# SUSTech-SLAM-XYZZY/SurfelMapping

Measured on AMD Instinct MI355X. Metric: frames/sec per GPU, 1242x375 KITTI-shaped RGB-D+semantic, full associate+fuse+merge, higher is better.
Workload: dtype f32; 1 GPU; BASELINE configs[1]: KITTI 1242x375 synthetic street sequence, 0.8 m/frame, depth noise 15.0 mm, metricise+conflict+cull+splat+associate+fuse+append per frame; frames=5..6245, multi_gpu=single stream, surfels_start=157613, surfels_end=5487352

## Files before the change

### surfelmapping_amd/csrc/sm_api.hip

```cpp
#include "sm_ctx.h"
#include "sm_kernels.h"

#include <hip/hip_runtime.h>

#include <dirent.h>
#include <link.h>

#include <algorithm>
#include <chrono>
#include <cmath>
#include <cstdio>
#include <cstdlib>
#include <cstring>
#include <atomic>
#include <functional>
#include <memory>
#include <mutex>
#include <string>
#include <thread>
#include <vector>

using namespace sm;

namespace {
// ... 91 lines not shown
        bool here = false;
        while (struct dirent *qe = readdir(qd)) {
            if (qe->d_name[0] < '0' || qe->d_name[0] > '9') continue;
            char gp[400];
            snprintf(gp, sizeof gp, "%s/%s/gpuid", qdir, qe->d_name);
            FILE *fg = fopen(gp, "r");
            unsigned long g = 0;
            if (fg) { if (fscanf(fg, "%lu", &g) == 1 && g == gpuid) here = true; fclose(fg); }
            if (here) break;
        }
        closedir(qd);
        if (here) ++procs;
    }
    closedir(pd);
    return procs;
}

bool gpu_shared_with_other_process(int dev)
{
    static std::mutex mu;
    static std::chrono::steady_clock::time_point last[MAX_DEV];
    static int cached[MAX_DEV];
    static bool valid[MAX_DEV] = {};
    if (dev < 0 || dev >= MAX_DEV) return false;
    std::lock_guard<std::mutex> lk(mu);
    const auto now = std::chrono::steady_clock::now();
    if (!valid[dev] || std::chrono::duration_cast<std::chrono::milliseconds>(now - last[dev]).count() > 1000) {
        cached[dev] = kfd_processes_on_gpu(dev);
        last[dev] = now; valid[dev] = true;
    }
    return cached[dev] > 1;
}

bool compaction_needs_tickets(const sm_ctx *s)
{
    const int dev = s->cfg.device;
    if (s->sw.compact_tickets >= 0) return s->sw.compact_tickets != 0;
    if (dev < 0 || dev >= MAX_DEV) return true;
    {
        std::lock_guard<std::mutex> lk(g_compact_mu);
        if (g_ctx_on_dev[dev] > 1) return true;
    }
    return gpu_shared_with_other_process(dev);
}

Switches read_switches()
{
    Switches sw;
    auto off = [](const char *name) { const char *e = std::getenv(name); return e && e[0] == '0'; };
    auto num = [](const char *name, long unset) { const char *e = std::getenv(name); return e ? std::atol(e) : unset; };
    sw.defer_assoc = !off("SM_DEFER_ASSOC");
    sw.two_launch = !off("SM_TWO_LAUNCH");
    sw.tail_squeeze = !off("SM_TAIL_SQUEEZE");
    sw.tail_thresh = (uint32_t)std::max(1l, num("SM_TAIL_THRESH", (long)TAIL_DEAD_THRESH));
    sw.pass_split = (int)num("SM_PASS_SPLIT", 0);
    if (const char *e = std::getenv("SM_PASS_TRACE")) { sw.trace = true; sw.trace_prefix = e; }
    if (std::getenv("SM_COMPACT_TICKETS")) sw.compact_tickets = off("SM_COMPACT_TICKETS") ? 0 : 1;
    sw.capacity_wait_us = num("SM_CAPACITY_WAIT_US", 2000);
    sw.check_alive = std::getenv("SM_CHECK_ALIVE") != nullptr;
    if (std::getenv("SM_PASS_WG_PER_CU")) sw.pass_wg_per_cu = (int)std::max(1l, num("SM_PASS_WG_PER_CU", 1));
    if (std::getenv("SM_COMPACT_WG_PER_CU")) sw.compact_wg_per_cu = (int)std::max(1l, num("SM_COMPACT_WG_PER_CU", 1));
    return sw;
}

void resident_grids(const Switches &sw, int device, int *pass_grid, int *compact_grid)
{
    int cus = 0, per_cu = 0;
    if (hipDeviceGetAttribute(&cus, hipDeviceAttributeMultiprocessorCount, device) != hipSuccess || cus <= 0) return;
    if (hipOccupancyMaxActiveBlocksPerMultiprocessor(&per_cu, k_surfel_pass<1>, 256, 0) == hipSuccess && per_cu > 0) {
        const int want = sw.pass_wg_per_cu ? sw.pass_wg_per_cu : std::max(1, per_cu - 1);
        *pass_grid = std::max(256, std::min(cus * want, MAX_GRID));
    }
    if (hipOccupancyMaxActiveBlocksPerMultiprocessor(&per_cu, k_compact<true>, 256, 0) == hipSuccess && per_cu > 0) {
        const int want = sw.compact_wg_per_cu ? std::min(per_cu, sw.compact_wg_per_cu) : std::min(per_cu, 4);
        *compact_grid = std::max(1, cus * want);
    }
}

int alloc_set(SetBufs &b, size_t cap)
{
    return dalloc(b.pos_conf, cap) || dalloc(b.norm_rad, cap) || dalloc(b.color, cap) || dalloc(b.init_time, cap) ||
           dalloc(b.time, cap) ? SM_E_HIP : SM_OK;
}

int grid_surfels(const sm_ctx *s)
{
    return (int)std::min<uint64_t>(std::max<uint64_t>(s->slots.tiles(), 1), MAX_GRID);
}

void check_alive(sm_ctx *s, uint32_t stage)
{
    if (!s->d_chk) return;
    hipLaunchKernelGGL(k_check_alive, dim3(64), dim3(256), 0, s->stream, s->d_state, s->d_alive, s->d_tile_dead, s->d_chk, stage);
}

int take_error(sm_ctx *s)
{
    if (s->h_state->error != 0) {
        const int e = s->h_state->error;
        s->h_state->error = 0;
        HIPCK(hipMemcpyAsync(&s->d_state->error, &s->h_state->error, sizeof(int32_t), hipMemcpyHostToDevice, s->stream));
        HIPCK(hipStreamSynchronize(s->stream));
        g_err = e == SM_E_CAPACITY ? "model capacity (MAX_VERTICES) exceeded; frame's new surfels dropped"
              : e == SM_E_UNSUPPORTED ? "unsupported operation flagged on the device"
              : "device-side error";
        return e;
    }
    return SM_OK;
}


static inline uint32_t assoc_wgs(const sm_ctx *s)
{
    return (uint32_t)(s->n_pix_blocks + 1) / 2u;
}

int launch_fixup(sm_ctx *s, const FrameParams &fp, const FixArgs &x)
{
    hipLaunchKernelGGL(k_pass_fixup, dim3(x.n_crew + 1), dim3(256), 0, s->stream, s->M, s->d_state, fp, x);
    HIPCK(hipGetLastError());
    return SM_OK;
}

int launch_assoc(sm_ctx *s, const AssocArgs &a, uint32_t stage)
{
    hipLaunchKernelGGL((k_associate_direct<false>), dim3(assoc_wgs(s)), dim3(PIX_BLOCK), 0, s->stream, a, ShardArgs{});
// ... 222 lines not shown
    fpc.compact_tickets = compaction_needs_tickets(s) ? 1 : 0;
    const auto compact = splat ? k_compact<true> : k_compact<false>;
    hipLaunchKernelGGL(compact, dim3(grid), dim3(256), 0, s->stream, s->M, s->d_state, fpc, s->d_cm,
                       s->d_dm, s->d_zm, s->d_tile_cnt, s->d_tile_allow, s->d_tile_keep, s->keyT(), s->d_tile_flag, epoch,
                       s->d_group_base, s->d_tb, s->cur().tile_flags, s->part.d_compact, s->d_alive, s->d_tile_dead);
    HIPCK(hipGetLastError());
    if (s->tl.mark(s->stream, 4, timed)) return SM_E_HIP;
    return SM_OK;
}

int launch_post_fill(sm_ctx *s)
{
    hipLaunchKernelGGL(k_post_fill, dim3(1024), dim3(256), 0, s->stream, s->d_state, s->d_alive, s->d_tile_dead);
    HIPCK(hipGetLastError());
    check_alive(s, 4u + 16u * (uint32_t)(s->tick & 0xFFFF));
    return SM_OK;
}

int ss_compact(sm_ctx *s);

int launch_associate_only(sm_ctx *s, const FrameParams &fp)
{
    hipLaunchKernelGGL(k_associate, dim3(s->n_pix_blocks), dim3(PIX_BLOCK), 0, s->stream, s->M, s->d_state, fp,
                       s->cur().depthT, s->cur().rgbsT, s->keyT(), s->d_xs, s->d_ys, s->d_validmask, s->d_fusedmask, s->d_blk_cnt, s->d_tb);
    HIPCK(hipGetLastError());
    return SM_OK;
}

int launch_associate(sm_ctx *s, const FrameParams &fp, bool timed)
{
    int rc = launch_associate_only(s, fp);
    if (rc) return rc;
    if (s->tl.mark(s->stream, 5, timed) || s->tl.mark(s->stream, 6, timed)) return SM_E_HIP;
    const PassPartials::Fold f = s->part.fold();
    hipLaunchKernelGGL(k_append_scan, dim3(s->n_pix_blocks), dim3(PIX_BLOCK), 0, s->stream, s->M, s->d_state, fp, s->cur().depthT,
                       s->cur().rgbsT, s->d_xs, s->d_ys, s->d_validmask, s->d_fusedmask, s->d_blk_cnt, s->d_log, s->d_tb, f.compact,
                       f.n_compact, s->d_alive, s->d_tile_dead, s->d_stat, f.lazy, f.fix, f.n_fix);
    s->part.clear();
    s->slots.append_enqueued();
    HIPCK(hipGetLastError());
    if (s->tl.mark(s->stream, 7, timed)) return SM_E_HIP;
    check_alive(s, 5u + 16u * (uint32_t)(s->tick & 0xFFFF));
    return SM_OK;
}

int launch_squeeze(sm_ctx *s, bool in_frame, bool tail, bool timed)
{
    FrameParams fp = make_params(s, s->curr_pose);
    fp.maintenance = in_frame ? 2 : 1;
    fp.compact_now = 1;
    fp.conflict_cap = 0xFFFFFFFFu;
    fp.no_masks = 1;
    fp.tail_thresh = tail ? s->sw.tail_thresh : 0u;
    const uint64_t tiles = s->slots.tiles() + 1;
    const int ngroups = std::max<int>(1, (int)((tiles + GROUP - 1) / GROUP));
    hipLaunchKernelGGL(k_scan_cull, dim3(ngroups), dim3(1024), 0, s->stream, s->d_state, s->d_tile_cnt, s->d_tile_allow,
                       s->d_tile_keep, s->d_group_tot, s->d_tile_dead, 1u, fp.tail_thresh);
    hipLaunchKernelGGL(k_cull_finalize, dim3(1), dim3(1024), 0, s->stream, s->d_state, fp, s->d_cm, s->d_dm, s->d_zm,
                       s->d_tile_cnt, s->d_tile_allow, s->d_tile_keep, s->d_group_tot, s->d_group_base, s->d_conf_part, 0u,
                       s->d_alive, s->d_tile_dead, s->d_stat);
    if (!in_frame && s->slots.keys_are_slots())
        hipLaunchKernelGGL(k_remap_keys, dim3((s->P + 255) / 256), dim3(256), 0, s->stream, s->d_state, s->keyT(), s->P, s->d_alive,
                           s->d_tile_keep, s->d_group_base);
    HIPCK(hipGetLastError());
    if (s->tl.mark(s->stream, 2, timed) || s->tl.mark(s->stream, 3, timed)) return SM_E_HIP;
    return launch_compact(s, fp, false, timed);
}

int discard_model(sm_ctx *s)
{
    int rc = pull_state(s);
    if (rc) return rc;
    if (s->h_state->count == 0 && !s->slots.maybe_garbage() && s->h_state->conflict_count == 0 && s->h_state->visible_count == 0) return SM_OK;
    if (s->slots.maybe_garbage()) {
        HIPCK(hipMemsetAsync(s->d_alive, 0xFF, s->alive_words * 8, s->stream));
        HIPCK(hipMemsetAsync(s->d_tile_dead, 0, s->dead_tiles * 4, s->stream));
        s->slots.model_discarded();
    }
    s->h_state->conflict_count = 0; s->h_state->visible_count = 0;
    return publish_dense(s, 0, 0);
}

void end_frame(sm_ctx *s, bool timed = true)
{
    if (s->cfg.preprocess) std::swap(s->d_lastT, s->d_filteredT);
    memcpy(s->last_pose, s->curr_pose, 64);
    s->tl.end_frame(timed);
    s->tick++;
}

int begin_frame(sm_ctx *s, const uint8_t *d_rgb, const uint16_t *d_raw, const uint8_t *d_sem, const float *pose, bool tile_flags, bool carry,
                FrameParams *fp_out, uint32_t *n_prep)
{
    if (s->pending_cull) { g_err = "sm_stage_conflict without sm_stage_cull"; return SM_E_ARG; }
    memcpy(s->curr_pose, pose, 64);
    s->trk.note_pose(pose);
    FrameParams fp = make_params(s, pose);
    const bool fusing = s->ref_set && s->tick != 0;
    int rc;
    if ((rc = s->tl.mark(s->stream, 8, fusing))) return rc;
    if ((rc = s->tl.mark(s->stream, 0, fusing))) return rc;
    const bool will_splat = fusing;
    s->plane_set ^= 1;
    fp.par = s->plane_set;
    if (s->defer_ok && will_splat) s->key_set ^= 1;
    ChainArgs ca{};
// ... 2 lines not shown
        ca.border = (int)std::ceil(s->cfg.stereo_border - 0.5f);
        ca.do_movings = s->ref_set ? 1 : 0;
        if (s->ref_set) {
            float linv[16];
            invert4(s->last_pose, linv);
            mul4(linv, s->curr_pose, ca.t_c2l.m);
        }
    }
    if ((rc = launch_prep(s, d_rgb, d_raw, d_sem, fp, will_splat, tile_flags, carry, s->cfg.preprocess ? &ca : nullptr)) < 0) return rc;
    *n_prep = (uint32_t)rc;
    if (!s->ref_set) {
        if (s->cfg.preprocess) std::swap(s->d_lastT, s->d_filteredT);
        memcpy(s->last_pose, s->curr_pose, 64);
        s->ref_set = true;
        s->tick++;
        return 0;
    }
    if ((rc = s->tl.mark(s->stream, 1, fusing))) return rc;
    s->raw_valid = true;
    s->raw_tick = s->tick;
    if (s->tick == 0) {
        fp.init_mode = 1;
        fp.log_frame = 0;
        if ((rc = discard_model(s))) return rc;
        s->part.clear();
        s->part.n_compact = 0;
        if ((rc = launch_associate(s, fp, false))) return rc;
        end_frame(s, false);
        return 0;
    }
    fp.splat_follows = 1;
    fp.log_frame = 1;
    *fp_out = fp;
    return 1;
}

int enqueue_frame(sm_ctx *s, const uint8_t *d_rgb, const uint16_t *d_raw, const uint8_t *d_sem, const float *pose)
{
    if (s->ss_on) { g_err = "context is configured for sharding: use the sm_shard_* entry points"; return SM_E_ARG; }
    FrameParams fp;
    const bool fusing = s->ref_set && s->tick != 0 && !s->pending_cull;
    using Due = sm_slots::SlotSchedule::Due;
    const Due due = fusing ? s->slots.decide_due() : Due::forced;
    const bool compact_now = due != Due::none;
    const bool squeeze = fusing && due == Due::period && s->sw.tail_squeeze && s->defer_ok;
    const bool carry = fusing && s->defer_ok;
    int rc = SM_OK;
    uint32_t n_prep = 0;
    if (!carry && (rc = complete_held(s, false))) return rc;
    rc = begin_frame(s, d_rgb, d_raw, d_sem, pose, fusing && (!compact_now || squeeze), carry, &fp, &n_prep);
    if (rc <= 0) return rc;
    fp.compact_now = compact_now && !squeeze ? 1u : 0u;
    if (squeeze) {
        if ((rc = complete_held(s, true))) return rc;
        if ((rc = launch_squeeze(s, true, true, true))) return rc;
        s->slots.squeezed_in_frame();
    } else
        s->slots.cull_noted(fp.compact_now != 0u);
    s->slots.keys_drawn(fp.compact_now == 0u);
    const bool one_pass = !fp.compact_now;
    Timeline::Flags &fl = s->tl.frame();
    fl.compacted = !one_pass || squeeze; fl.one_pass = fl.direct = one_pass; fl.squeezed = squeeze;
    if (one_pass) {
        if ((rc = launch_surfel_pass(s, fp, true, true, n_prep, squeeze))) return rc;
        if ((rc = launch_associate_direct(s, fp, true))) return rc;
        end_frame(s);
        return SM_OK;
    }
    if ((rc = launch_conflict(s, fp, true))) return rc;
    if ((rc = launch_compact(s, fp, true, true))) return rc;
    if ((rc = launch_associate(s, fp, true))) return rc;
    end_frame(s);
    return SM_OK;
}

int upload_inputs(sm_ctx *s, const uint8_t *rgb, const uint16_t *depth, const uint8_t *sem)
{
    const size_t P = (size_t)s->P;
    hipStream_t st = s->stream;
    if (rgb) HIPCK(hipMemcpyAsync(s->d_rgb, rgb, P * 3, hipMemcpyHostToDevice, st));
    if (depth) HIPCK(hipMemcpyAsync(s->d_depth_raw, depth, P * 2, hipMemcpyHostToDevice, st));
    if (sem) HIPCK(hipMemcpyAsync(s->d_sem, sem, P, hipMemcpyHostToDevice, st));
    return SM_OK;
}

int alloc_frame_set(sm_ctx *s, FrameSet &f)
{
    auto get = [s](auto *&p, size_t n, bool zero) -> int {
        Dev<void> m;
        const size_t bytes = std::max<size_t>(n, 1) * sizeof *p;
        HIPCK(hipMalloc(m.put(), bytes));
        if (zero) HIPCK(hipMemset(m, 0, bytes));
        p = static_cast<std::remove_reference_t<decltype(p)>>(m.get());
        s->frame_mem.push_back(std::move(m));
        return SM_OK;
    };
    const size_t P = (size_t)s->P;
    return get(f.depthT, P, true) || get(f.rgbsT, P, true) || get(f.dcT, P, true) || get(f.tile_flags, s->tb_tiles, true) ||
           get(f.wave_cnt, s->dead_tiles, false) || get(f.prep_part, 256, false) ? SM_E_HIP : SM_OK;
}

int alloc_ctx(sm_ctx *s)
{
    const size_t P = (size_t)s->P, cap = s->cap, nwords = s->alive_words, ntiles = s->dead_tiles, tb = s->tb_tiles;
    if (hipStreamCreateWithFlags(s->stream.put(), hipStreamNonBlocking) != hipSuccess ||
        alloc_set(s->m_bufs[0], cap) ||
        dalloc(s->d_state, 1) || dalloc(s->d_log, FRAME_LOG_LEN) || hipHostMalloc(s->h_state.put(), sizeof(DevState), hipHostMallocDefault) != hipSuccess ||
        hipHostMalloc(s->h_stat.put(), 8, hipHostMallocMapped) != hipSuccess || hipHostGetDevicePointer((void **)&s->d_stat, s->h_stat, 0) != hipSuccess ||
        dalloc(s->d_filteredT, P) || dalloc(s->d_lastT, P) ||
        alloc_frame_set(s, s->fset[0]) || dalloc(s->d_key[0], P) ||
        (s->defer_ok && (alloc_frame_set(s, s->fset[1]) || dalloc(s->d_key[1], P))) ||
        dalloc(s->d_rgb, P * 3) || dalloc(s->d_sem, P) || dalloc(s->d_depth_raw, P) || dalloc(s->d_depth_f32, P) ||
        dalloc(s->d_xs, (size_t)s->W * 2) || dalloc(s->d_ys, (size_t)s->H * 2) ||
        dalloc(s->d_cm, nwords) || dalloc(s->d_dm, nwords) || dalloc(s->d_zm, nwords) ||
        dalloc(s->d_alive, nwords) || hipMemset(s->d_alive, 0xFF, nwords * 8) != hipSuccess ||
        dalloc(s->d_tile_dead, ntiles) || hipMemset(s->d_tile_dead, 0, ntiles * 4) != hipSuccess ||
        dalloc(s->d_tile_cnt, ntiles * 3) || dalloc(s->d_tile_allow, ntiles) || dalloc(s->d_tile_keep, ntiles) || dalloc(s->d_tile_flag, ntiles) ||
        hipMemset(s->d_tile_flag, 0, ntiles * 4) != hipSuccess ||
        dalloc(s->d_group_tot, (ntiles / GROUP + 2) * 4) || dalloc(s->d_group_base, ntiles / GROUP + 2) ||
        dalloc(s->d_conf_part, (size_t)MAX_GRID * 4) || dalloc(s->part.d_compact, (size_t)MAX_GRID) || dalloc(s->part.d_lazy, (size_t)MAX_GRID) ||
        dalloc(s->part.d_fix, (size_t)MAX_GRID * 2 + 2) || dalloc(s->d_undo, cap + TILE) ||
        dalloc(s->d_conf_sub, (size_t)2 * SUB_SET) || hipMemset(s->d_conf_sub, 0, (size_t)2 * SUB_SET * 4) != hipSuccess ||
        dalloc(s->d_tb, tb * 8) ||
        dalloc(s->d_validmask, (P + 63) / 64 + 4) || dalloc(s->d_fusedmask, (P + 63) / 64 + 4) || dalloc(s->d_blk_cnt, (size_t)s->n_pix_blocks) ||
        dalloc(s->d_blk_cand, (size_t)s->n_grp * CAND_GROUP_MAX) || dalloc(s->d_grp_cand, (size_t)s->n_grp) ||
        dalloc(s->d_frame_sub, (size_t)6 * SUB_SET) || hipMemset(s->d_frame_sub, 0, (size_t)6 * SUB_SET * 4) != hipSuccess)
        return SM_E_HIP;
    s->M.s[0] = s->m_bufs[0].view();
    *s->h_stat = 0ull;
    for (int i = 0; i < 2; ++i) { s->fset[i].nf_sub = s->d_frame_sub + (2 + 2 * i) * SUB_SET; s->fset[i].conf_sub = s->d_conf_sub + i * SUB_SET; }
    if (!s->defer_ok) s->alias_frame_sets();
    return SM_OK;
}

}


void sm_impl::invert4(const float *m, float *out)
{
    float a[16];
    a[0] = m[5] * m[10] * m[15] - m[5] * m[11] * m[14] - m[9] * m[6] * m[15] + m[9] * m[7] * m[14] +
           m[13] * m[6] * m[11] - m[13] * m[7] * m[10];
    a[4] = -m[4] * m[10] * m[15] + m[4] * m[11] * m[14] + m[8] * m[6] * m[15] - m[8] * m[7] * m[14] -
           m[12] * m[6] * m[11] + m[12] * m[7] * m[10];
    a[8] = m[4] * m[9] * m[15] - m[4] * m[11] * m[13] - m[8] * m[5] * m[15] + m[8] * m[7] * m[13] +
           m[12] * m[5] * m[11] - m[12] * m[7] * m[9];
    a[12] = -m[4] * m[9] * m[14] + m[4] * m[10] * m[13] + m[8] * m[5] * m[14] - m[8] * m[6] * m[13] -
            m[12] * m[5] * m[10] + m[12] * m[6] * m[9];
    a[1] = -m[1] * m[10] * m[15] + m[1] * m[11] * m[14] + m[9] * m[2] * m[15] - m[9] * m[3] * m[14] -
           m[13] * m[2] * m[11] + m[13] * m[3] * m[10];
    a[5] = m[0] * m[10] * m[15] - m[0] * m[11] * m[14] - m[8] * m[2] * m[15] + m[8] * m[3] * m[14] +
           m[12] * m[2] * m[11] - m[12] * m[3] * m[10];
    a[9] = -m[0] * m[9] * m[15] + m[0] * m[11] * m[13] + m[8] * m[1] * m[15] - m[8] * m[3] * m[13] -
           m[12] * m[1] * m[11] + m[12] * m[3] * m[9];
    a[13] = m[0] * m[9] * m[14] - m[0] * m[10] * m[13] - m[8] * m[1] * m[14] + m[8] * m[2] * m[13] +
            m[12] * m[1] * m[10] - m[12] * m[2] * m[9];
    a[2] = m[1] * m[6] * m[15] - m[1] * m[7] * m[14] - m[5] * m[2] * m[15] + m[5] * m[3] * m[14] +
           m[13] * m[2] * m[7] - m[13] * m[3] * m[6];
    a[6] = -m[0] * m[6] * m[15] + m[0] * m[7] * m[14] + m[4] * m[2] * m[15] - m[4] * m[3] * m[14] -
           m[12] * m[2] * m[7] + m[12] * m[3] * m[6];
    a[10] = m[0] * m[5] * m[15] - m[0] * m[7] * m[13] - m[4] * m[1] * m[15] + m[4] * m[3] * m[13] +
            m[12] * m[1] * m[7] - m[12] * m[3] * m[5];
    a[14] = -m[0] * m[5] * m[14] + m[0] * m[6] * m[13] + m[4] * m[1] * m[14] - m[4] * m[2] * m[13] -
            m[12] * m[1] * m[6] + m[12] * m[2] * m[5];
    a[3] = -m[1] * m[6] * m[11] + m[1] * m[7] * m[10] + m[5] * m[2] * m[11] - m[5] * m[3] * m[10] -
           m[9] * m[2] * m[7] + m[9] * m[3] * m[6];
    a[7] = m[0] * m[6] * m[11] - m[0] * m[7] * m[10] - m[4] * m[2] * m[11] + m[4] * m[3] * m[10] +
           m[8] * m[2] * m[7] - m[8] * m[3] * m[6];
    a[11] = -m[0] * m[5] * m[11] + m[0] * m[7] * m[9] + m[4] * m[1] * m[11] - m[4] * m[3] * m[9] -
// ... 929 lines not shown
```

### surfelmapping_amd/csrc/sm_ctx.h

```cpp
#pragma once

#include "../../include/sm_c_api.h"
#include "sm_device.h"
#include "sm_slots.h"

#include <hip/hip_runtime.h>

#include <algorithm>
#include <cassert>
#include <cmath>
#include <cstdio>
#include <cstring>
#include <functional>
#include <map>
#include <memory>
#include <string>
#include <utility>
#include <vector>

namespace sm { struct TrackState; struct TrackRgbState; struct RenderParams; struct ViewParams; struct ViewShade; struct RecallChunk; struct WarpChunk; }

namespace sm_impl __attribute__((visibility("hidden"))) {

using namespace sm;
// ... 154 lines not shown
    size_t cand_cap = 0;
    Event ev[2];
};

struct Lidar {
    Dev<float> d_dir, d_el;
    std::vector<float> key;
    Dev<uint8_t> d_poses;
    size_t pose_cap = 0;
    Dev<uint8_t> d_tally;
    Event ev[2];
    sm_lidar_stats_t stats{};
    bool stats_valid = false;
};

struct Place {
    bool on = false;
    sm_fern_params p{};
    Dev<uint4> d_table;
    Dev<uint8_t> d_rgb;
    Dev<uint16_t> d_depth;
    Dev<uint32_t> d_code;
    Dev<uint32_t> d_codes;
    Dev<int32_t> d_times;
    size_t cap = 0;
    std::vector<float> poses;
    std::vector<int32_t> times;
    Dev<unsigned long long> d_keys;
    Dev<uint32_t> d_dis;
    size_t dis_cap = 0;
    uint32_t count() const { return (uint32_t)times.size(); }
    bool timed = false;
    Event ev[4];
    bool auto_on = false;
    sm_auto_place_params ap{};
    int64_t rest_until = 0;
    sm_auto_place_stats_t stats{};
};

struct AutoLoop {
    bool on = false;
    bool search = false;
    sm_search_params sp{};
    sm_auto_loop_params p{};
    std::vector<std::string> paths;
    int64_t rest_until = 0;
    sm_auto_loop_stats_t stats{};
};

struct Switches {
    bool defer_assoc = true;
    bool two_launch = true;
    bool tail_squeeze = true;
    uint32_t tail_thresh = 0;
    int pass_split = 0;
    bool trace = false;
    std::string trace_prefix;
    int compact_tickets = -1;
    long capacity_wait_us = 2000;
    bool check_alive = false;
    int pass_wg_per_cu = 0;
    int compact_wg_per_cu = 0;
};

class HeldBack {
public:
    void hold_fixup(const FixArgs &x) { assert(!has_fix_ && !has_assoc_); fix_ = x; has_fix_ = true; }
    void hold_assoc(const AssocArgs &a) { assoc_ = a; has_assoc_ = true; }
    AssocArgs *take_assoc(FixArgs *&fix)
    {
        assert(has_assoc_ || !has_fix_);
        fix = std::exchange(has_fix_, false) ? &fix_ : nullptr;
        return std::exchange(has_assoc_, false) ? &assoc_ : nullptr;
    }
    void hold_settle(const ShardSettle &ss) { settle_ = ss; has_settle_ = true; }
    ShardSettle *take_settle() { return std::exchange(has_settle_, false) ? &settle_ : nullptr; }
    void hold_stats(uint32_t *nf) { nf_ = nf; }
    uint32_t *take_stats() { return std::exchange(nf_, nullptr); }
private:
    bool has_fix_ = false, has_assoc_ = false, has_settle_ = false;
    FixArgs fix_{};
    AssocArgs assoc_{};
    ShardSettle settle_{};
    uint32_t *nf_ = nullptr;
};

struct FrameSet {
    float *depthT = nullptr;
    uint32_t *rgbsT = nullptr;
    uint2 *dcT = nullptr;
    uint8_t *tile_flags = nullptr;
    uint4 *wave_cnt = nullptr;
    uint2 *prep_part = nullptr;
    uint32_t *nf_sub = nullptr;
    uint32_t *conf_sub = nullptr;
};

struct PassPartials {
    Dev<uint2> d_compact;
    Dev<uint4> d_lazy;
    Dev<uint2> d_fix;
    int fix_set = 0;
    uint32_t n_compact = 0;
    uint32_t n_fix = 0;
    bool pass_live = false;
    void clear() { pass_live = false; }
// ... 9 lines not shown
    uint64_t frames = 0, read = 0;
    int mark(hipStream_t st, int which, bool timed)
    {
        if (timed && ev) HIPCK(hipEventRecord(ev[which][frames % EV_RING], st));
        return SM_OK;
    }
    Flags &frame() { return flags[frames % EV_RING]; }
    void end_frame(bool timed) { if (timed && ev) frames++; }
};

}

using namespace sm_impl;

struct sm_ctx {
    Stream stream;
    Stream stream_in;
    sm_config cfg{};
    int W = 0, H = 0, P = 0;
    uint32_t cap = 0;
    int plane_set = 0;
    FrameSet fset[2];
    const FrameSet &cur() const { return fset[plane_set]; }
    const FrameSet &prev() const { return fset[plane_set ^ 1]; }
    void alias_frame_sets() { uint32_t *c = fset[1].conf_sub; fset[1] = fset[0]; fset[1].conf_sub = c; }
    Dev<uint64_t> d_key[2];
    int key_set = 0;
    uint64_t *keyT() const { return d_key[key_set]; }
    std::vector<Dev<void>> frame_mem;
    Model M{};
    SetBufs m_bufs[2];
    Dev<DevState> d_state;
    Host<DevState> h_state;
    Dev<float> d_filteredT, d_lastT;
    Dev<uint8_t> d_rgb, d_sem;
    Dev<uint16_t> d_depth_raw;
    static constexpr int IN_RING = 3;
    struct InSlot { Dev<uint8_t> rgb; uint8_t *sem = nullptr; uint16_t *depth = nullptr;
                    Host<unsigned char> h_stage; Event ev_in, ev_free; bool used = false; };
    InSlot in[IN_RING];
    size_t in_off_depth = 0, in_off_sem = 0, in_bytes = 0;
    uint32_t in_next = 0;
    const uint16_t *in_last_depth = nullptr; const uint8_t *in_last_sem = nullptr;
    int in_depth_slot = -1, in_sem_slot = -1;
    std::vector<std::pair<Host<unsigned char>, size_t>> pinned;
    Dev<float> d_depth_f32;
    Dev<float> d_xs, d_ys;
    float h_wtab[169];
    Dev<uint64_t> d_cm, d_dm, d_zm;
    Dev<uint32_t> d_tile_cnt, d_tile_allow, d_tile_keep, d_tile_flag;
    Dev<uint32_t> d_group_tot, d_group_base;
    Dev<uint64_t> d_alive;
    Dev<uint32_t> d_tile_dead;
    size_t alive_words = 0, dead_tiles = 0;
    sm_slots::SlotSchedule slots;
    Host<unsigned long long> h_stat; unsigned long long *d_stat = nullptr;
    Dev<uint32_t> d_tb;
    Dev<uint32_t> d_conf_part;
    PassPartials part;
    Dev<float> d_undo;
    int fix_grid = 128;
    Dev<uint32_t> d_blk_cand, d_grp_cand;
    Dev<uint32_t> d_frame_sub;
    uint32_t n_grp = 0, cand_group = 16;
    Dev<unsigned long long> d_pass_trace;
    int pass_trace_grid = 0;
    Dev<unsigned long long> d_ap_trace;
    int ap_trace_n[4] = {0, 0, 0, 0};
    Dev<uint32_t> d_conf_sub;
    uint32_t n_conf_part = 0;
    uint32_t tb_tiles = 0;
    int compact_grid = COMPACT_GRID;
    int pass_grid = MAX_GRID;
    Dev<uint64_t> d_validmask, d_fusedmask;
    Dev<uint2> d_blk_cnt;
    bool ss_on = false;
    bool rig_on = false;
    float rig_last_time = -1.0e30f;
    int ss_rank = 0, ss_world = 1;
    uint32_t ss_frames = 0;
    sm_collective_fn ss_coll = nullptr;
    void *ss_user = nullptr;
    void *ss_comm = nullptr;
    Dev<uint64_t> d_galive, d_new_alive, d_gmask;
    Dev<uint32_t> d_chk;
    Dev<uint64_t> d_capx;
    Dev<uint32_t> d_ss_info;
    Switches sw;
    bool defer_ok = false;
    HeldBack held;
    static constexpr uint32_t N_CREW = 32;
    int n_pix_blocks = 0;
    Dev<void> d_export;
    size_t export_bytes = 0;
    ModelView rm;
    Tracker trk;
    Retire ret;
    RenderMaps maps;
    Recall rec;
    Warp warp;
    AutoLoop aloop;
    Search srch;
    Lidar lid;
    Place place;
    int tick = 0;
    bool ref_set = false;
// ... 117 lines not shown
```

### surfelmapping_amd/csrc/sm_device.h

```cpp
#pragma once

#include <hip/hip_runtime.h>
#include <stdint.h>

namespace sm {

constexpr uint64_t KEY_EMPTY = 0x7FFFFFFFFFFFFFFFull;
constexpr int TILE = 1024;
constexpr int TILE_WORDS = TILE / 64;
constexpr int PIX_BLOCK = 256;
constexpr int SUB_STRIDE = 32;
constexpr int SUB_SET = 64 * SUB_STRIDE;

struct SurfelSet {
    float4 *pos_conf;
    float4 *norm_rad;
    uint32_t *color;
    float *init_time;
    float *time;
};

struct Model {
    SurfelSet s[2];
};

struct DevState {
    uint32_t count;
    uint32_t offset;
    uint32_t cur;
    uint32_t cull_n;
    uint32_t cull_src, cull_dst;
    uint32_t n_kill;
    uint32_t conflict_count;
    uint32_t data_count, unstable_count, fused_count;
    uint32_t visible_count;
    uint32_t append_n;
    int32_t error;
    uint32_t frames_logged;
    uint32_t n_static;
    uint32_t n_conf_skipped;
    uint32_t n_splat_skipped;
    uint32_t garbage;
    uint32_t garbage_prev;
    uint32_t do_compact;
    uint32_t cap_binds;
    uint32_t first_moving;
    uint32_t compact_ticket;
    uint32_t stat_frames;
    uint32_t first_live;
    uint32_t fl_dirty2[2];
    uint32_t slow_frames;
    uint32_t slow_done[2];
    uint32_t pend;
    uint32_t pend_tick;
    uint32_t holes_last;
    uint32_t sq_static;
    uint32_t sq_tail, sq_full;
};

struct FrameLog { uint32_t tick, n_before, n_after_cull, n_kill, conflict_count, visible_count, fused_count, unstable_count, n_static, n_conf_skipped, n_splat_skipped, n_slots; };
constexpr uint32_t FRAME_LOG_LEN = 1024;

struct FrameParams {
    float pose[16];
    float t_inv[16];
    float fx, fy, cx, cy;
    float inv_fx, inv_fy;
    float cols, rows;
    int W, H, P;
    float min_depth, max_depth;
    float conflict_thresh;
    float fuse_thresh;
    float stereo_border;
    int is_clean;
    int time;
    int time_delta;
    float depth_cutoff;
    uint32_t conflict_cap;
    int splat_follows;
    int log_frame;
    uint32_t max_vertices;
    int init_mode;
    float inv_fx_fb, inv_fy_fb;
    int use_bounds;
    uint32_t compact_now;
    int maintenance;
    int no_masks;
    uint32_t tail_thresh;
    int compact_tickets;
    int no_exempt;
    int shard_slots;
    int par;
};

__device__ __forceinline__ float min_glsl(float a, float b) { return (b < a) ? b : a; }

__device__ __forceinline__ int tex_idx(float t, int n)
{
    float f = floorf(t * (float)n);
    if (!(f >= 0.0f)) return 0;
    if (f > (float)(n - 1)) return n - 1;
    return (int)f;
}

__device__ __forceinline__ float3 xform3(const float *m, float x, float y, float z)
{
    float3 r;
    r.x = ((m[0] * x + m[4] * y) + m[8] * z) + m[12];
    r.y = ((m[1] * x + m[5] * y) + m[9] * z) + m[13];
    r.z = ((m[2] * x + m[6] * y) + m[10] * z) + m[14];
// ... 349 lines not shown
```

### surfelmapping_amd/csrc/sm_k_cull.h

```cpp
#pragma once

#ifndef SM_CONFLICT_WAVES
#define SM_CONFLICT_WAVES 5
#endif
__global__ __launch_bounds__(256) __attribute__((amdgpu_waves_per_eu(SM_CONFLICT_WAVES, 8))) void k_conflict(Model M, const DevState *__restrict__ st, FrameParams fp,
                                                  const uint2 *__restrict__ dcT ,
                                                  uint64_t *__restrict__ cm, uint64_t *__restrict__ dm,
                                                  uint64_t *__restrict__ zm, uint32_t *__restrict__ tile_cnt,
                                                  const uint32_t *__restrict__ tb, uint8_t *__restrict__ tile_flags,
                                                  uint32_t *__restrict__ blk_part ,
                                                  const uint64_t *__restrict__ alive,
                                                  uint32_t *__restrict__ conf_sub )
{
    __shared__ uint32_t s_red[4][3];
    __shared__ uint64_t s_m[3][TILE_WORDS];
    __shared__ uint8_t s_flags[64];
    const uint32_t N = st->count;
    const bool has_dead = st->garbage != 0u;
    const uint32_t exempt = fp.no_exempt ? 0xFFFFFFFFu : st->first_live;
    const float4 *__restrict__ pc = M.s[st->cur].pos_conf;
    const uint32_t ntiles = (N + TILE - 1) / TILE;
    const int lane = threadIdx.x & 63, wave = threadIdx.x >> 6;
    uint32_t skipped = 0;
    uint32_t acc = 0;
// ... 575 lines not shown
            if (threadIdx.x < 8) atomicExch(&tb[(size_t)tile * 8 + threadIdx.x], 0u);
            asm volatile("s_waitcnt vmcnt(0)" ::: "memory");
            __syncthreads();
            if (threadIdx.x == 0) {
                __hip_atomic_exchange(&tile_flag[tile], epoch, __ATOMIC_RELAXED, __HIP_MEMORY_SCOPE_AGENT);
                if (kcount && base_id != tile * TILE) {
                    const uint32_t first = base_id / TILE;
                    const uint32_t last = min(tile - 1u, (base_id + kcount - 1u) / TILE);
                    for (uint32_t t = first; t <= last; ++t) {
                        uint32_t spins = 0;
                        while (__hip_atomic_load(&tile_flag[t], __ATOMIC_RELAXED, __HIP_MEMORY_SCOPE_AGENT) != epoch) {
                            __builtin_amdgcn_s_sleep(2);
                            if (++spins > (1u << 24)) { st->error = -6; break; }
                        }
                    }
                }
            }
            __syncthreads();
            if (in_frame) {
                if (threadIdx.x < TILE_WORDS && (uint64_t)(tile * TILE_WORDS + threadIdx.x) * 64u < N) alive[tile * TILE_WORDS + threadIdx.x] = ~0ull;
                if (threadIdx.x == 0) { tile_dead[tile] = 0u; tile_flags[tile] = 0; }
            }
#pragma unroll
            for (int r = 0; r < 4; ++r) {
                if (kept[r]) {
                    set.pos_conf[nid[r]] = v[r];
                    set.norm_rad[nid[r]] = nr[r];
                    set.color[nid[r]] = col[r];
                    set.init_time[nid[r]] = it[r];
                    set.time[nid[r]] = tl[r];
                }
                bounds_expand_wave(tb, kept[r], nid[r] / (uint32_t)TILE, v[r].x, v[r].y, v[r].z, tl[r], false);
            }
        }
        if (SPLAT) {
#pragma unroll
            for (int r = 0; r < 4; ++r) {
                bool drew = false;
                if (kept[r])
                    drew = splat_one(fp, v[r].x, v[r].y, v[r].z, tl[r], nid[r], keyT);
                vis += (uint32_t)__popcll(__ballot(drew));
            }
        }
        __syncthreads();
    }
    if (SPLAT) {
        if (lane == 0) s_vis[wave] = vis;
        __syncthreads();
        if (threadIdx.x == 0)
            blk_part[blockIdx.x] = make_uint2(s_vis[0] + s_vis[1] + s_vis[2] + s_vis[3], skipped);
    }
}

__global__ __launch_bounds__(256) void k_cull_lazy(Model M, const DevState *__restrict__ st, FrameParams fp,
                                                   const uint64_t *__restrict__ cm, const uint64_t *__restrict__ dm,
                                                   const uint64_t *__restrict__ zm, const uint32_t *__restrict__ tile_cnt,
                                                   const uint32_t *__restrict__ tile_allow,
                                                   uint64_t *__restrict__ alive, uint32_t *__restrict__ tile_dead)
{
    const uint32_t N = st->cull_n;
    const SurfelSet set = M.s[st->cull_src];
    const uint32_t ntiles = (N + TILE - 1) / TILE;
    const int lane = threadIdx.x & 63, wave = threadIdx.x >> 6;
    const bool had_dead = st->garbage_prev != 0u, cap_binds = st->cap_binds != 0u;
    uint32_t iter = 0;
    uint32_t m_nconf = 0, m_nkill = 0, m_dead = 0;
    for (uint32_t tile = blockIdx.x; tile < ntiles; tile += gridDim.x, ++iter) {
        if ((iter & 63u) == 0u) {
            const uint64_t tl = (uint64_t)tile + (uint64_t)lane * gridDim.x;
            const bool in = tl < ntiles;
            const uint32_t tt = in ? (uint32_t)tl : 0u;
            m_nconf = tile_cnt[tt * 3]; m_nkill = tile_cnt[tt * 3 + 1];
            m_dead = had_dead ? tile_dead[tt] : 0u;
        }
        const int sl = (int)(iter & 63u);
        const uint32_t nconf = lane_bcast(m_nconf, sl), nkill = lane_bcast(m_nkill, sl);
        const uint32_t tdead = lane_bcast(m_dead, sl);
        const bool touched = nconf != 0u || nkill != 0u;
        if (!touched) continue;
        float4 pv[4];
#pragma unroll
        for (int r = 0; r < 4; ++r) {
            const uint32_t kc = min((tile * TILE_WORDS + r * 4 + wave) * 64u + lane, N - 1u);
            pv[r] = set.pos_conf[kc];
        }
        const uint32_t allow = (touched && cap_binds) ? tile_allow[tile] : nconf;
        uint32_t killed = 0;
#pragma unroll
        for (int r = 0; r < 4; ++r) {
            const int w = r * 4 + wave;
            const uint32_t word = tile * TILE_WORDS + (uint32_t)w;
            const uint32_t k = word * 64u + lane;
            const uint64_t base = (uint64_t)word * 64u;
            uint64_t range = 0ull;
            if (base < N) { const uint64_t rem = (uint64_t)N - base; range = rem >= 64 ? ~0ull : ((1ull << rem) - 1ull); }
            const uint64_t valid = range & ((tdead != 0u) ? alive[word] : ~0ull);
            uint64_t keep = valid, ce = 0ull;
            if (touched) {
                ce = cm[word];
                if (allow != nconf) {
                    uint32_t before = 0;
                    for (int x = 0; x < w; ++x) before += (uint32_t)__popcll(cm[tile * TILE_WORDS + x]);
                    ce = before >= allow ? 0ull : first_n_bits(ce, allow - before);
                }
                keep = ~(zm[word] | (ce & dm[word])) & valid;
                if (keep != valid && lane == 0) alive[word] = keep | ~range;
// ... 49 lines not shown
```

### surfelmapping_amd/csrc/sm_kernels.h

```cpp
#pragma once

#include "sm_device.h"

namespace sm {

#include "sm_k_prep.h"
#include "sm_k_cull.h"
#include "sm_k_pass.h"
#include "sm_k_assoc.h"
#include "sm_k_shard.h"

}
```

Before: 26350 frames/s.

## Fuse in-frame tail squeeze scan, cull finalize and compaction into one kernel

Adds a k_squeeze kernel that does the dead-tile prefix scan, the squeeze plan decision and the in-place compaction in one launch. Each block recomputes the per-tile dead prefix redundantly in LDS. Blocks order themselves with per-tile epoch flags and spin waits, and the last block finishes the frame bookkeeping. This replaces the scan_cull, cull_finalize and compact launch chain on in-frame squeeze frames, and lets the held frame completion skip its separate finalize. The aim is to cut launch count and global round trips, at the cost of redundant scanning per block, a large LDS footprint that may lower occupancy, and spin-wait deadlock risk. The compact grid is also capped by k_squeeze occupancy.

```diff
diff --git a/surfelmapping_amd/csrc/sm_api.hip b/surfelmapping_amd/csrc/sm_api.hip
--- a/surfelmapping_amd/csrc/sm_api.hip
+++ b/surfelmapping_amd/csrc/sm_api.hip
@@ -167,6 +167,7 @@
     sw.defer_assoc = !off("SM_DEFER_ASSOC");
     sw.two_launch = !off("SM_TWO_LAUNCH");
     sw.tail_squeeze = !off("SM_TAIL_SQUEEZE");
+    sw.squeeze_fused = !off("SM_SQUEEZE_FUSED");
     sw.tail_thresh = (uint32_t)std::max(1l, num("SM_TAIL_THRESH", (long)TAIL_DEAD_THRESH));
     sw.pass_split = (int)num("SM_PASS_SPLIT", 0);
     if (const char *e = std::getenv("SM_PASS_TRACE")) { sw.trace = true; sw.trace_prefix = e; }
@@ -187,6 +188,8 @@
         *pass_grid = std::max(256, std::min(cus * want, MAX_GRID));
     }
     if (hipOccupancyMaxActiveBlocksPerMultiprocessor(&per_cu, k_compact<true>, 256, 0) == hipSuccess && per_cu > 0) {
+        int per_cu_sq = 0;
+        if (hipOccupancyMaxActiveBlocksPerMultiprocessor(&per_cu_sq, k_squeeze, 256, 0) == hipSuccess && per_cu_sq > 0) per_cu = std::min(per_cu, per_cu_sq);
         const int want = sw.compact_wg_per_cu ? std::min(per_cu, sw.compact_wg_per_cu) : std::min(per_cu, 4);
         *compact_grid = std::max(1, cus * want);
     }
@@ -515,6 +518,18 @@
     fp.conflict_cap = 0xFFFFFFFFu;
     fp.no_masks = 1;
     fp.tail_thresh = tail ? s->sw.tail_thresh : 0u;
+    if (in_frame && s->sw.squeeze_fused) {
+        if (s->tl.mark(s->stream, 2, timed) || s->tl.mark(s->stream, 3, timed)) return SM_E_HIP;
+        s->part.clear();
+        const int grid = std::min(grid_surfels(s), s->compact_grid);
+        const uint32_t epoch = s->slots.next_cull_epoch();
+        fp.compact_tickets = compaction_needs_tickets(s) ? 1 : 0;
+        uint32_t *nf = s->held.take_stats();
+        hipLaunchKernelGGL(k_squeeze, dim3(grid), dim3(256), 0, s->stream, s->M, s->d_state, fp, s->d_tile_flag, epoch, s->d_tb,
+                           s->cur().tile_flags, s->d_alive, s->d_tile_dead, s->d_sq_sub, nf, s->part.fix_cur(), s->part.n_fix, s->d_log, s->d_stat);
+        HIPCK(hipGetLastError());
+        return s->tl.mark(s->stream, 4, timed) ? SM_E_HIP : SM_OK;
+    }
     const uint64_t tiles = s->slots.tiles() + 1;
     const int ngroups = std::max<int>(1, (int)((tiles + GROUP - 1) / GROUP));
     hipLaunchKernelGGL(k_scan_cull, dim3(ngroups), dim3(1024), 0, s->stream, s->d_state, s->d_tile_cnt, s->d_tile_allow,
@@ -623,7 +638,7 @@
     if (rc <= 0) return rc;
     fp.compact_now = compact_now && !squeeze ? 1u : 0u;
     if (squeeze) {
-        if ((rc = complete_held(s, true))) return rc;
+        if ((rc = complete_held(s, !s->sw.squeeze_fused))) return rc;
         if ((rc = launch_squeeze(s, true, true, true))) return rc;
         s->slots.squeezed_in_frame();
     } else
@@ -686,6 +701,7 @@
         dalloc(s->d_cm, nwords) || dalloc(s->d_dm, nwords) || dalloc(s->d_zm, nwords) ||
         dalloc(s->d_alive, nwords) || hipMemset(s->d_alive, 0xFF, nwords * 8) != hipSuccess ||
         dalloc(s->d_tile_dead, ntiles) || hipMemset(s->d_tile_dead, 0, ntiles * 4) != hipSuccess ||
+        dalloc(s->d_sq_sub, (size_t)SUB_SET) || hipMemset(s->d_sq_sub, 0, (size_t)SUB_SET * 4) != hipSuccess ||
         dalloc(s->d_tile_cnt, ntiles * 3) || dalloc(s->d_tile_allow, ntiles) || dalloc(s->d_tile_keep, ntiles) || dalloc(s->d_tile_flag, ntiles) ||
         hipMemset(s->d_tile_flag, 0, ntiles * 4) != hipSuccess ||
         dalloc(s->d_group_tot, (ntiles / GROUP + 2) * 4) || dalloc(s->d_group_base, ntiles / GROUP + 2) ||
diff --git a/surfelmapping_amd/csrc/sm_ctx.h b/surfelmapping_amd/csrc/sm_ctx.h
--- a/surfelmapping_amd/csrc/sm_ctx.h
+++ b/surfelmapping_amd/csrc/sm_ctx.h
@@ -230,6 +230,7 @@
     bool defer_assoc = true;
     bool two_launch = true;
     bool tail_squeeze = true;
+    bool squeeze_fused = true;
     uint32_t tail_thresh = 0;
     int pass_split = 0;
     bool trace = false;
@@ -345,6 +346,7 @@
     Dev<uint32_t> d_group_tot, d_group_base;
     Dev<uint64_t> d_alive;
     Dev<uint32_t> d_tile_dead;
+    Dev<uint32_t> d_sq_sub;
     size_t alive_words = 0, dead_tiles = 0;
     sm_slots::SlotSchedule slots;
     Host<unsigned long long> h_stat; unsigned long long *d_stat = nullptr;
diff --git a/surfelmapping_amd/csrc/sm_device.h b/surfelmapping_amd/csrc/sm_device.h
--- a/surfelmapping_amd/csrc/sm_device.h
+++ b/surfelmapping_amd/csrc/sm_device.h
@@ -56,6 +56,8 @@
     uint32_t holes_last;
     uint32_t sq_static;
     uint32_t sq_tail, sq_full;
+    uint32_t sq_done;
+    uint32_t sq_ticket;
 };
 
 struct FrameLog { uint32_t tick, n_before, n_after_cull, n_kill, conflict_count, visible_count, fused_count, unstable_count, n_static, n_conf_skipped, n_splat_skipped, n_slots; };
diff --git a/surfelmapping_amd/csrc/sm_k_cull.h b/surfelmapping_amd/csrc/sm_k_cull.h
--- a/surfelmapping_amd/csrc/sm_k_cull.h
+++ b/surfelmapping_amd/csrc/sm_k_cull.h
@@ -651,6 +651,223 @@
     }
 }
 
+constexpr uint32_t SQ_SLAB = 8192;
+static_assert(TAIL_GARBAGE_DIV == sm_squeeze::GARBAGE_DIV, "one garbage rule");
+
+__device__ __forceinline__ void finalize_frame(DevState *__restrict__ st, uint32_t *__restrict__ nf, const uint2 *__restrict__ fix_prev,
+                                               uint32_t n_fix_prev, FrameLog *__restrict__ log, uint32_t *s_red);
+
+__global__ __launch_bounds__(256) void k_squeeze(Model M, DevState *__restrict__ st, FrameParams fp,
+                                                 uint32_t *__restrict__ tile_flag, uint32_t epoch,
+                                                 uint32_t *__restrict__ tb, uint8_t *__restrict__ tile_flags,
+                                                 uint64_t *__restrict__ alive, uint32_t *__restrict__ tile_dead,
+                                                 uint32_t *__restrict__ done_sub ,
+                                                 uint32_t *__restrict__ nf, const uint2 *__restrict__ fix_prev, uint32_t n_fix_prev,
+                                                 FrameLog *__restrict__ log, unsigned long long *__restrict__ host_stat)
+{
+    __shared__ uint32_t s_slab[SQ_SLAB];
+    __shared__ uint32_t s_pre[sm_squeeze::THREADS];
+    __shared__ uint32_t s_wsum[4], s_first, s_dense, s_left, s_tk, s_last, s_red[16];
+    __shared__ uint64_t s_keep[TILE_WORDS];
+    __shared__ uint32_t s_kpre[TILE_WORDS + 1];
+    const uint32_t N = st->count;
+    const SurfelSet set = M.s[st->cur];
+    const uint32_t ntiles = (N + TILE - 1) / TILE;
+    const int lane = threadIdx.x & 63, wave = threadIdx.x >> 6;
+    const uint32_t C = sm_squeeze::chunk_len(ntiles);
+    const uint32_t t0 = min(threadIdx.x * C, ntiles), t1 = min(t0 + C, ntiles);
+    sm_squeeze::Chunk ch = sm_squeeze::chunk_empty();
+    if (threadIdx.x == 0) { s_first = sm_squeeze::NONE; s_dense = sm_squeeze::NONE; s_left = 0u; }
+    for (uint32_t s0 = 0; s0 < ntiles; s0 += SQ_SLAB) {
+        const uint32_t s1 = min(s0 + SQ_SLAB, ntiles);
+        {
+            uint32_t d[SQ_SLAB / 256];
+#pragma unroll
+            for (int u = 0; u < (int)(SQ_SLAB / 256); ++u) d[u] = tile_dead[min(s0 + (uint32_t)u * 256u + threadIdx.x, ntiles - 1u)];
+#pragma unroll
+            for (int u = 0; u < (int)(SQ_SLAB / 256); ++u) {
+                const uint32_t i = s0 + (uint32_t)u * 256u + threadIdx.x;
+                if (i < s1) s_slab[i - s0] = d[u];
+            }
+        }
+        __syncthreads();
+        for (uint32_t t = max(t0, s0); t < min(t1, s1); ++t) {
+            const uint32_t d = s_slab[t - s0];
+            s_slab[t - s0] = ch.dead;
+            sm_squeeze::chunk_add(ch, t, d, fp.tail_thresh);
+        }
+        __syncthreads();
+    }
+    const uint32_t slab0 = ntiles ? ((ntiles - 1u) / SQ_SLAB) * SQ_SLAB : 0u;
+    uint32_t inc = ch.dead;
+#pragma unroll
+    for (int o = 1; o < 64; o <<= 1) {
+        const uint32_t x = __shfl_up(inc, o);
+        if (lane >= o) inc += x;
+    }
+    if (lane == 63) s_wsum[wave] = inc;
+    __syncthreads();
+    uint32_t pre = inc - ch.dead;
+    for (int w = 0; w < wave; ++w) pre += s_wsum[w];
+    s_pre[threadIdx.x] = pre;
+    if (ch.first_dead != sm_squeeze::NONE) atomicMin(&s_first, ch.first_dead);
+    if (ch.first_dense != sm_squeeze::NONE) atomicMin(&s_dense, ch.first_dense);
+    __syncthreads();
+    sm_squeeze::Totals tot;
+    tot.dead = s_wsum[0] + s_wsum[1] + s_wsum[2] + s_wsum[3];
+    tot.first_dead = s_first; tot.first_dense = s_dense;
+    if (tot.first_dense != sm_squeeze::NONE && ch.first_dense == tot.first_dense) s_left = pre + ch.dead_below_dense;
+    __syncthreads();
+    tot.dead_below_dense = s_left;
+    const sm_squeeze::Plan plan = sm_squeeze::decide(N, (uint32_t)TILE, fp.tail_thresh, tot);
+    const uint32_t lo = plan.bnd;
+    const bool use_tickets = fp.compact_tickets != 0;
+    uint32_t rr_tile = lo + blockIdx.x, iter = 0, m_base = 0;
+    for (;;) {
+        uint32_t tile, base_id;
+        if (!use_tickets) {
+            tile = rr_tile;
+            if (tile >= ntiles) break;
+            if ((iter & 63u) == 0u) {
+                const uint64_t tl = (uint64_t)tile + (uint64_t)lane * gridDim.x;
+                if (tl < ntiles) {
+                    const uint32_t t = (uint32_t)tl;
+                    const uint32_t below = t >= slab0 ? s_pre[t / C] + s_slab[t - slab0] : sm_squeeze::dead_below(s_pre, C, t, tile_dead);
+                    m_base = sm_squeeze::tile_base(plan, t, (uint32_t)TILE, below);
+                }
+            }
+            base_id = lane_bcast(m_base, (int)(iter & 63u));
+            rr_tile += gridDim.x; ++iter;
+        } else {
+            __syncthreads();
+            if (threadIdx.x == 0) s_tk = atomicAdd(&st->sq_ticket, 1u);
+            __syncthreads();
+            tile = lo + s_tk;
+            if (tile >= ntiles) break;
+            uint32_t in;
+            if (tile >= slab0) in = s_slab[tile - slab0];
+            else {
+                uint32_t x_in = 0;
+                for (uint32_t x = (tile / C) * C + (uint32_t)lane; x < tile; x += 64u) x_in += tile_dead[x];
+                in = wave_sum_u32(x_in);
+            }
+            base_id = sm_squeeze::tile_base(plan, tile, (uint32_t)TILE, s_pre[tile / C] + in);
+        }
+        float4 v[4], nr[4];
+        uint32_t col[4], nid[4];
+        float it[4], tl[4];
+        bool kept[4];
+#pragma unroll
+        for (int r = 0; r < 4; ++r) {
+            const uint32_t k = (tile * TILE_WORDS + r * 4 + wave) * 64u + lane;
+            const uint32_t kc = min(k, N - 1u);
+            v[r] = set.pos_conf[kc];
+            tl[r] = set.time[kc];
+            const float4 n4 = set.norm_rad[kc];
+            nr[r] = make_float4(n4.x, n4.y, n4.z, n4.w); col[r] = set.color[kc]; it[r] = set.init_time[kc];
+        }
+        if (threadIdx.x < TILE_WORDS) {
+            const uint32_t word = tile * TILE_WORDS + threadIdx.x;
+            const uint64_t base = (uint64_t)word * 64u;
+            uint64_t keep = 0;
+            if (base < N) {
+                const uint64_t rem = (uint64_t)N - base;
+                keep = (rem >= 64 ? ~0ull : ((1ull << rem) - 1ull)) & alive[word];
+            }
+            s_keep[threadIdx.x] = keep;
+        }
+        __syncthreads();
+        if (threadIdx.x <= TILE_WORDS) {
+            uint32_t before = 0;
+            for (int w = 0; w < (int)threadIdx.x; ++w) before += (uint32_t)__popcll(s_keep[w]);
+            s_kpre[threadIdx.x] = before;
+        }
+        __syncthreads();
+        const uint32_t kcount = s_kpre[TILE_WORDS];
+#pragma unroll
+        for (int r = 0; r < 4; ++r) {
+            const int w = r * 4 + wave;
+            const uint64_t keepw = s_keep[w];
+            kept[r] = (keepw >> lane) & 1ull;
+            nid[r] = base_id + s_kpre[w] + (uint32_t)__popcll(keepw & ((1ull << lane) - 1ull));
+        }
+        if (threadIdx.x < 8) atomicExch(&tb[(size_t)tile * 8 + threadIdx.x], 0u);
+        asm volatile("s_waitcnt vmcnt(0)" ::: "memory");
+        __syncthreads();
+        if (threadIdx.x == 0) {
+            __hip_atomic_exchange(&tile_flag[tile], epoch, __ATOMIC_RELAXED, __HIP_MEMORY_SCOPE_AGENT);
+            if (kcount && base_id != tile * TILE) {
+                const uint32_t first = base_id / TILE;
+                const uint32_t last = min(tile - 1u, (base_id + kcount - 1u) / TILE);
+                for (uint32_t t = first; t <= last; ++t) {
+                    uint32_t spins = 0;
+                    while (__hip_atomic_load(&tile_flag[t], __ATOMIC_RELAXED, __HIP_MEMORY_SCOPE_AGENT) != epoch) {
+                        __builtin_amdgcn_s_sleep(2);
+                        if (++spins > (1u << 24)) { st->error = -6; break; }
+                    }
+                }
+            }
+        }
+        __syncthreads();
+        if (threadIdx.x < TILE_WORDS && (uint64_t)(tile * TILE_WORDS + threadIdx.x) * 64u < N) alive[tile * TILE_WORDS + threadIdx.x] = ~0ull;
+        if (threadIdx.x == 0) tile_flags[tile] = 0;
+#pragma unroll
+        for (int r = 0; r < 4; ++r) {
+            if (kept[r]) {
+                set.pos_conf[nid[r]] = v[r];
+                set.norm_rad[nid[r]] = nr[r];
+                set.color[nid[r]] = col[r];
+                set.init_time[nid[r]] = it[r];
+                set.time[nid[r]] = tl[r];
+            }
+            bounds_expand_wave(tb, kept[r], nid[r] / (uint32_t)TILE, v[r].x, v[r].y, v[r].z, tl[r], false);
+        }
+        __syncthreads();
+    }
+    asm volatile("s_waitcnt vmcnt(0)" ::: "memory");
+    __syncthreads();
+    if (threadIdx.x == 0) {
+        uint32_t last = 0u;
+        const uint32_t j = blockIdx.x & 63u;
+        const uint32_t mine = (gridDim.x - j + 63u) / 64u;
+        if (__hip_atomic_fetch_add(&done_sub[j * SUB_STRIDE], 1u, __ATOMIC_RELAXED, __HIP_MEMORY_SCOPE_AGENT) + 1u == mine)
+            last = __hip_atomic_fetch_add(&st->sq_done, 1u, __ATOMIC_RELAXED, __HIP_MEMORY_SCOPE_AGENT) + 1u == min(gridDim.x, 64u) ? 1u : 0u;
+        s_last = last;
+    }
+    __syncthreads();
+    if (s_last == 0u) return;
+    if (nf) finalize_frame(st, nf, fix_prev, n_fix_prev, log, s_red);
+    for (uint32_t t = plan.bnd + threadIdx.x; t < ntiles; t += 256u) tile_dead[t] = 0u;
+    if (threadIdx.x < 64) done_sub[threadIdx.x * SUB_STRIDE] = 0u;
+    if (threadIdx.x == 0) {
+        const uint32_t g0 = st->garbage;
+        const uint32_t holes = st->holes_last;
+        const uint32_t old_first = st->first_live, old_offset = st->offset;
+        const bool tail = sm_squeeze::is_tail(plan);
+        st->cull_n = N;
+        st->cull_src = st->cur;
+        st->cull_dst = st->cur;
+        st->garbage_prev = g0;
+        st->cap_binds = 0u;
+        st->do_compact = 1u;
+        st->first_moving = plan.bnd;
+        st->sq_static = plan.bnd < ntiles ? plan.nstatic + 1u : 0u;
+        if (tail) st->sq_tail = st->sq_tail + 1u; else st->sq_full = st->sq_full + 1u;
+        st->compact_ticket = 0u;
+        st->first_live = tail ? old_first : 0u;
+        st->fl_dirty2[0] = 0u; st->fl_dirty2[1] = 0u;
+        st->slow_done[0] = 0u; st->slow_done[1] = 0u;
+        st->holes_last = 0u;
+        st->count = plan.kept + plan.left;
+        st->offset = old_offset - (g0 - holes) + plan.left;
+        st->garbage = plan.left;
+        st->sq_done = 0u; st->sq_ticket = 0u;
+        if (host_stat)
+            __hip_atomic_store(host_stat, ((unsigned long long)st->stat_frames << 32) | (unsigned long long)(plan.kept + plan.left),
+                               __ATOMIC_RELAXED, __HIP_MEMORY_SCOPE_SYSTEM);
+    }
+}
+
 __global__ __launch_bounds__(256) void k_cull_lazy(Model M, const DevState *__restrict__ st, FrameParams fp,
                                                    const uint64_t *__restrict__ cm, const uint64_t *__restrict__ dm,
                                                    const uint64_t *__restrict__ zm, const uint32_t *__restrict__ tile_cnt,
diff --git a/surfelmapping_amd/csrc/sm_kernels.h b/surfelmapping_amd/csrc/sm_kernels.h
--- a/surfelmapping_amd/csrc/sm_kernels.h
+++ b/surfelmapping_amd/csrc/sm_kernels.h
@@ -1,6 +1,7 @@
 #pragma once
 
 #include "sm_device.h"
+#include "sm_squeeze_plan.h"
 
 namespace sm {
 
diff --git a/surfelmapping_amd/csrc/sm_squeeze_plan.h b/surfelmapping_amd/csrc/sm_squeeze_plan.h
--- /dev/null
+++ b/surfelmapping_amd/csrc/sm_squeeze_plan.h
@@ -0,0 +1,95 @@
+#pragma once
+
+#include <stdint.h>
+
+#if defined(__HIPCC__)
+#define SM_SQ_HD __host__ __device__ __forceinline__
+#else
+#define SM_SQ_HD inline
+#endif
+
+namespace sm_squeeze {
+
+constexpr uint32_t THREADS = 256;
+constexpr uint32_t NONE = 0xFFFFFFFFu;
+constexpr uint32_t GARBAGE_DIV = 32;
+
+SM_SQ_HD uint32_t tiles_of(uint32_t n, uint32_t tile) { return n / tile + (n % tile ? 1u : 0u); }
+SM_SQ_HD uint32_t chunk_len(uint32_t ntiles) { const uint32_t c = (ntiles + THREADS - 1u) / THREADS; return c ? c : 1u; }
+
+struct Chunk {
+    uint32_t dead;
+    uint32_t first_dead;
+    uint32_t first_dense;
+    uint32_t dead_below_dense;
+};
+
+SM_SQ_HD Chunk chunk_empty() { return Chunk{0u, NONE, NONE, 0u}; }
+
+SM_SQ_HD void chunk_add(Chunk &c, uint32_t t, uint32_t dead, uint32_t thresh)
+{
+    if (dead != 0u && c.first_dead == NONE) c.first_dead = t;
+    if (thresh != 0u && dead >= thresh && c.first_dense == NONE) { c.first_dense = t; c.dead_below_dense = c.dead; }
+    c.dead += dead;
+}
+
+SM_SQ_HD Chunk chunk_scan(uint32_t thread, uint32_t chunk, uint32_t ntiles, const uint32_t *tile_dead, uint32_t thresh)
+{
+    Chunk c = chunk_empty();
+    const uint64_t t0 = (uint64_t)thread * chunk;
+    for (uint64_t t = t0; t < t0 + chunk && t < ntiles; ++t) chunk_add(c, (uint32_t)t, tile_dead[t], thresh);
+    return c;
+}
+
+struct Totals {
+    uint32_t dead;
+    uint32_t first_dead;
+    uint32_t first_dense;
+    uint32_t dead_below_dense;
+};
+
+struct Plan {
+    uint32_t ntiles;
+    uint32_t bnd;
+    uint32_t left;
+    uint32_t kept;
+    uint32_t nstatic;
+};
+
+SM_SQ_HD bool is_tail(const Plan &p) { return p.left != 0u; }
+
+SM_SQ_HD Plan decide(uint32_t n, uint32_t tile, uint32_t thresh, const Totals &t)
+{
+    Plan p;
+    p.ntiles = tiles_of(n, tile);
+    p.kept = n - t.dead;
+    p.left = 0u;
+    const bool any = t.first_dead != NONE && t.first_dead < p.ntiles;
+    p.bnd = any ? t.first_dead : p.ntiles;
+    p.nstatic = any ? (uint32_t)(((uint64_t)t.first_dead * tile < n) ? t.first_dead * tile : n) : n;
+    if (thresh != 0u) {
+        const uint32_t bt = t.first_dense < p.ntiles ? t.first_dense : p.ntiles;
+        const uint32_t left = bt < p.ntiles ? t.dead_below_dense : t.dead;
+        if (!(left == 0u || left > n / GARBAGE_DIV)) {
+            p.left = left;
+            p.bnd = bt;
+            p.nstatic = ((uint64_t)bt * tile < n) ? bt * tile : n;
+        }
+    }
+    return p;
+}
+
+SM_SQ_HD uint32_t dead_below(const uint32_t *chunk_pre , uint32_t chunk, uint32_t t, const uint32_t *tile_dead)
+{
+    const uint32_t c = t / chunk;
+    uint32_t d = chunk_pre[c];
+    for (uint32_t x = c * chunk; x < t; ++x) d += tile_dead[x];
+    return d;
+}
+
+SM_SQ_HD uint32_t tile_base(const Plan &p, uint32_t t, uint32_t tile, uint32_t dead_below_t)
+{
+    return t * tile - dead_below_t + p.left;
+}
+
+}
```

Result: no change. 26140 frames/s (-0.8%).
